# ethan-li-coding/AD-Census

Hardware: AMD Instinct MI355X
Metric: stereo pairs/s at 1920x1080 D=128 (ADCensusStereo::Match, images and disparity map resident in HBM) (higher is better)
Workload: dtype f32; 1 GPU; noise 1920x1080 D=128 (BASELINE.json configs[3]); batch=160 distinct pairs (seeds 12345+i), 668 per GPU (cycled), queue=static round-robin partition, in_flight_per_gpu=1, parallelism=replicas x1 (independent pairs), full=False

## Files before the change

adcensus_amd/__init__.py:

```python
import ctypes as C
import os

import numpy as np

_HERE = os.path.dirname(os.path.abspath(__file__))
LIB_PATH = os.environ.get("ADC_HIP_LIB") or os.path.join(_HERE, "lib", "libadcensus_hip.so")

STAGES = ["cost", "arms", "aggregate", "scanline", "wta", "refine"]
(BUF_GRAY_LEFT, BUF_GRAY_RIGHT, BUF_CENSUS_LEFT, BUF_CENSUS_RIGHT, BUF_ARMS, BUF_SUPCOUNT_H, BUF_SUPCOUNT_V,
 BUF_VOLUME_A, BUF_DISP_LEFT, BUF_DISP_RIGHT, BUF_OUTLIER_LABEL) = range(11)
(RUN_GRAY_CENSUS, RUN_COST, RUN_ARMS, RUN_AGGREGATE, RUN_SCANLINE, RUN_WTA, RUN_LRCHECK, RUN_REGION_VOTING,
 RUN_INTERPOLATION, RUN_DISCONTINUITY, RUN_MEDIAN) = range(11)
MAX_DISP_RANGE = 2047
PAPER_CENSUS5X5, PAPER_SO_SUM, PAPER_RIGHT_ARMS = 1, 2, 4
LR_CONSISTENT, LR_MISMATCH, LR_OCCLUSION = 0, 1, 2
FILL_WTA, FILL_VOTING, FILL_INTERPOLATION, FILL_NONE = 0, 1, 2, 3
PROV_LR_MASK, PROV_FILL_SHIFT = 3, 2
PROV_SPECKLE = 0x10
PIX_BGR8, PIX_RGB8, PIX_GRAY8, PIX_BGRA8 = 0, 1, 2, 3
PIX_GRAY16 = 0x10
PIX_BAYER_RGGB8, PIX_BAYER_GRBG8, PIX_BAYER_GBRG8, PIX_BAYER_BGGR8 = 0x20, 0x21, 0x22, 0x23
PIX_BAYER_RGGB16, PIX_BAYER_GRBG16, PIX_BAYER_GBRG16, PIX_BAYER_BGGR16 = 0x30, 0x31, 0x32, 0x33
PIX_YUYV, PIX_UYVY, PIX_NV12 = 0x40, 0x41, 0x42
PIX_BYTES = {PIX_BGR8: 3, PIX_RGB8: 3, PIX_GRAY8: 1, PIX_BGRA8: 4, PIX_GRAY16: 2, PIX_YUYV: 2, PIX_UYVY: 2, PIX_NV12: 1,
# ... 325 lines not shown
    L.adc_get_aggregate_info.restype = C.c_int
    L.adc_get_aggregate_kernel.argtypes = [vp]
    L.adc_get_aggregate_kernel.restype = C.c_char_p
    L.adc_host_register.argtypes = [vp, C.c_size_t]
    L.adc_host_register.restype = C.c_int
    L.adc_host_unregister.argtypes = [vp]
    L.adc_host_unregister.restype = C.c_int
    L.adc_set_paper_modes.argtypes = [vp, C.c_uint32]
    L.adc_set_paper_modes.restype = C.c_int
    L.adc_get_stream.argtypes = [vp]
    L.adc_get_stream.restype = vp
    L.adc_device_synchronize.restype = C.c_int
    L.adc_device_malloc.argtypes = [C.c_size_t]
    L.adc_device_malloc.restype = vp
    L.adc_device_free.argtypes = [vp]
    L.adc_device_free.restype = None
    L.adc_memcpy_h2d.argtypes = [vp, vp, C.c_size_t]
    L.adc_memcpy_h2d.restype = C.c_int
    L.adc_memcpy_d2h.argtypes = [vp, vp, C.c_size_t]
    L.adc_memcpy_d2h.restype = C.c_int
    L.adc_device_copy_ms.argtypes = [vp, vp, C.c_size_t, C.c_int]
    L.adc_device_copy_ms.restype = C.c_double
    if hasattr(L, "adc_device_copy_kernel_ms"):
        L.adc_device_copy_kernel_ms.argtypes = [vp, vp, C.c_size_t, C.c_int]
        L.adc_device_copy_kernel_ms.restype = C.c_double
    L.adc_debug_read.argtypes = [vp, C.c_int, vp]
    L.adc_debug_read.restype = C.c_int
    L.adc_debug_write.argtypes = [vp, C.c_int, vp]
    L.adc_debug_write.restype = C.c_int
    L.adc_debug_set_images.argtypes = [vp, u8p, u8p]
    L.adc_debug_set_images.restype = C.c_int
    L.adc_debug_run.argtypes = [vp, C.c_int, C.c_int]
    L.adc_debug_run.restype = C.c_int
    L.adc_farm_create.argtypes = [i32, i32, C.POINTER(ADCensusOption), C.c_int, C.c_int]
    L.adc_farm_create.restype = vp
    L.adc_farm_destroy.argtypes = [vp]
    L.adc_farm_destroy.restype = None
    L.adc_farm_submit.argtypes = [vp, u8p, u8p, vp, C.POINTER(C.c_uint64)]
    L.adc_farm_submit.restype = C.c_int
    L.adc_farm_wait.argtypes = [vp, C.c_uint64]
    L.adc_farm_wait.restype = C.c_int
    L.adc_farm_drain.argtypes = [vp]
    L.adc_farm_drain.restype = C.c_int64
    L.adc_debug_counter.argtypes = [vp, C.c_int]
    L.adc_debug_counter.restype = C.c_int64
    L.adc_debug_voting_stats.argtypes = [vp, C.POINTER(C.c_int64), C.POINTER(C.c_int64)]
    L.adc_debug_voting_stats.restype = C.c_int
    _lib = L
    return L


def device_count():
    return lib().adc_device_count()


def last_error():
    return lib().adc_last_error().decode()


def host_register(arr):
    if lib().adc_host_register(arr.ctypes.data, arr.nbytes) != 0:
        raise RuntimeError("adc_host_register failed: " + last_error())


def host_unregister(arr):
    lib().adc_host_unregister(arr.ctypes.data)
# ... 523 lines not shown
            raise RuntimeError("adc_set_paper_modes failed: " + last_error())

    def aggregate_kernel(self):
        return lib().adc_get_aggregate_kernel(self._h).decode()

    def _buf_spec(self, which):
        h, w, d = self.height, self.width, self.disp_range
        return {
            BUF_GRAY_LEFT: (np.uint8, (h, w)), BUF_GRAY_RIGHT: (np.uint8, (h, w)),
            BUF_CENSUS_LEFT: (np.uint64, (h, w)), BUF_CENSUS_RIGHT: (np.uint64, (h, w)),
            BUF_ARMS: (np.uint8, (h, w, 4)),
            BUF_SUPCOUNT_H: (np.uint16, (h, w)), BUF_SUPCOUNT_V: (np.uint16, (h, w)),
            BUF_VOLUME_A: (np.float32, (h, w, d)),
            BUF_DISP_LEFT: (np.float32, (h, w)), BUF_DISP_RIGHT: (np.float32, (h, w)),
            BUF_OUTLIER_LABEL: (np.uint8, (h, w)),
        }[which]

    def debug_read(self, which):
        dt, shp = self._buf_spec(which)
        out = np.empty(shp, dtype=dt)
        rc = lib().adc_debug_read(self._h, which, out.ctypes.data)
        if rc != 0:
            raise RuntimeError("adc_debug_read(%d) failed: %s" % (which, last_error()))
        return out

    def debug_write(self, which, arr):
        dt, shp = self._buf_spec(which)
        a = np.ascontiguousarray(arr, dtype=dt)
        assert a.shape == tuple(shp), (a.shape, shp)
        rc = lib().adc_debug_write(self._h, which, a.ctypes.data)
        if rc != 0:
            raise RuntimeError("adc_debug_write(%d) failed: %s" % (which, last_error()))

    def debug_set_images(self, img_left, img_right):
        l, r = _img(img_left), _img(img_right)
        if lib().adc_debug_set_images(self._h, l.ctypes.data, r.ctypes.data) != 0:
            raise RuntimeError("adc_debug_set_images failed: " + last_error())

    def debug_run(self, stage, arg=0):
        rc = lib().adc_debug_run(self._h, stage, arg)
        if rc != 0:
            raise RuntimeError("adc_debug_run(%d) failed: %s" % (stage, last_error()))

    def debug_set_budget(self, kernels):
        rc = lib().adc_debug_run(self._h, RUN_REGION_VOTING, -int(kernels))
        if rc != 0:
            raise RuntimeError("adc_debug_run failed: " + last_error())

    def debug_counter(self, which):
        return int(lib().adc_debug_counter(self._h, which))

    def voting_stats(self):
        r, e = C.c_int64(0), C.c_int64(0)
        lib().adc_debug_voting_stats(self._h, C.byref(r), C.byref(e))
        return int(r.value), int(e.value)
```

adcensus_amd/csrc/capi.hip:

```cpp
#include "adc_internal.h"
#include "adc_device_fn.h"
#include "itp_plan.h"

#include <math.h>
#include <stdio.h>
#include <stdlib.h>
#include <string.h>
#include <string>
#include <vector>
#include <new>
#include <mutex>
#include <atomic>

static thread_local std::string g_last_error;

#ifdef ADC_FAULT_INJECTION
static std::atomic<long> g_fi_calls{0};
static std::atomic<long> g_fi_fail_at{[] { const char* e = getenv("ADC_TEST_FAIL_AT"); return e ? atol(e) : 0L; }()};
extern "C" int adc_test_fault_now(void) { const long n = ++g_fi_calls; return n == g_fi_fail_at.load(); }
extern "C" void adc_test_fail_at(long n) { g_fi_calls = 0; g_fi_fail_at = n; }
extern "C" long adc_test_hip_calls(void) { return g_fi_calls.load(); }
static std::atomic<long> g_fi_live{0};
extern "C" long adc_test_live_buffers(void) { return g_fi_live.load(); }
#define ADC_LIVE(d) (g_fi_live += (d))
// ... 1847 lines not shown
    case ADC_BUF_DISP_LEFT: return {h->disp_l, P * 4, false};
    case ADC_BUF_DISP_RIGHT: return {h->disp_r, P * 4, false};
    case ADC_BUF_OUTLIER_LABEL: return {h->label, P, false};
    default: return {nullptr, 0, false};
    }
}

int adc_debug_read(adc_handle* h, int which, void* dst)
{
    if (!h || !dst) return 1;
    hipSetDevice(h->device);
    const BufDesc b = buf_desc(h, which);
    if (!b.ptr) return 1;
    if (b.volume) {
        if (adc_launch_unpad_volume(h, h->vol_a, h->vol_b) != hipSuccess) return 2;
        if (hipMemcpyAsync(dst, h->vol_b, b.bytes, hipMemcpyDeviceToHost, h->stream) != hipSuccess) return 2;
    } else if (hipMemcpyAsync(dst, b.ptr, b.bytes, hipMemcpyDeviceToHost, h->stream) != hipSuccess) return 2;
    return hipStreamSynchronize(h->stream) == hipSuccess ? 0 : 2;
}

int adc_debug_write(adc_handle* h, int which, const void* src)
{
    if (!h || !src) return 1;
    hipSetDevice(h->device);
    const BufDesc b = buf_desc(h, which);
    if (!b.ptr) return 1;
    if (b.volume) {
        if (hipMemcpyAsync(h->vol_b, src, b.bytes, hipMemcpyHostToDevice, h->stream) != hipSuccess) return 2;
        if (adc_launch_pad_volume(h, h->vol_b, h->vol_a) != hipSuccess) return 2;
    } else if (hipMemcpyAsync(b.ptr, src, b.bytes, hipMemcpyHostToDevice, h->stream) != hipSuccess) return 2;
    return hipStreamSynchronize(h->stream) == hipSuccess ? 0 : 2;
}

int adc_debug_set_images(adc_handle* h, const uint8_t* left, const uint8_t* right)
{
    if (!h || !left || !right) return 1;
    hipSetDevice(h->device);
    const size_t P = (size_t)h->p.W * h->p.H;
    images_own(h, true);
    if (hipMemcpy(h->img_l, left, P * 3, hipMemcpyHostToDevice) != hipSuccess) return 2;
    if (hipMemcpy(h->img_r, right, P * 3, hipMemcpyHostToDevice) != hipSuccess) return 2;
    return 0;
}

int adc_debug_run(adc_handle* h, int stage, int arg)
{
    if (!h) return 1;
    hipSetDevice(h->device);
    hipError_t e = hipSuccess;
    bool fuse_cost = false; AggArms arms = AGG_ARMS_UNKNOWN;
    switch (stage) {
    case ADC_RUN_GRAY_CENSUS: e = adc_launch_gray_census(h); break;
    case ADC_RUN_COST: e = adc_launch_cost(h, h->vol_a); break;
    case ADC_RUN_ARMS: e = adc_launch_arms(h); break;
    case ADC_RUN_AGGREGATE:
        e = hipMemsetAsync(h->armmax + ADC_NZ_BASE, 0, 2 * ADC_NZ_SHARDS * ADC_NZ_STRIDE * sizeof(int), h->heavy);
        if (e == hipSuccess) e = adc_launch_records(h);
        if (e == hipSuccess && arg >= 200) {
            int am[2] = {0, 0};
            e = hipMemcpy(am, h->armmax, 2 * sizeof(int), hipMemcpyDeviceToHost);
            if (e == hipSuccess) learn_take_arms(&h->learned, am);
            if (e == hipSuccess) arms = AGG_ARMS_EXACT;
            if (e == hipSuccess && h->pin_nz) e = hipMemcpyAsync(h->pin_nz, h->armmax + ADC_NZ_BASE, 2 * ADC_NZ_SHARDS * ADC_NZ_STRIDE * sizeof(int32_t), hipMemcpyDeviceToHost, h->heavy);
            if (e == hipSuccess && h->pin_nz) e = hipStreamSynchronize(h->heavy);
            if (e == hipSuccess && h->pin_nz) {
                long long nz[2];
// ... 108 lines not shown
```

adcensus_amd/csrc/k_refine.hip:

```cpp
#include "adc_internal.h"
#include <mutex>
#include "adc_device_fn.h"
#include "itp_plan.h"

#include <vector>
#include <stdio.h>
#include <stdlib.h>

__device__ __forceinline__ bool lr_invalid(const float* __restrict__ dl, const float* __restrict__ dr, int W, int x, int y,
                                           float thres, int& col_right, float& disp_r)
{
    const float d = dl[(size_t)y * W + x];
    col_right = -1;
    disp_r = 0.f;
    if (d == ADC_INVALID_FLOAT) return true;
    const long cr = lroundf((float)x - d);
    if (cr < 0 || cr >= W) return true;
    col_right = (int)cr;
    disp_r = dr[(size_t)y * W + cr];
    return fabsf(d - disp_r) > thres;
}

__global__ __launch_bounds__(256) void k_lr_phase1(const float* __restrict__ dl, const float* __restrict__ dr,
                                                   uint8_t* __restrict__ inv, int W, int H, float thres)
// ... 157 lines not shown
        if (mismatch) {
            int key = (hit != ADC_INVALID_FLOAT && dist < 9999) ? dist * 16 + s : 0x7fffffff;
            float val = hit;
#pragma unroll
            for (int msk = 8; msk >= 1; msk >>= 1) {
                const int ok = __shfl_xor(key, msk, 64);
                const float ov = __shfl_xor(val, msk, 64);
                if (ok < key) { key = ok; val = ov; }
            }
            unsigned long long hb = __ballot(hit != ADC_INVALID_FLOAT);
            any = ((hb >> (lane & 48)) & 0xffffull) != 0;
            best = key != 0x7fffffff ? val : 0.0f;
        } else {
            float val = hit;
#pragma unroll
            for (int msk = 8; msk >= 1; msk >>= 1) {
                const float ov = __shfl_xor(val, msk, 64);
                val = ov < val ? ov : val;
            }
            any = val != ADC_INVALID_FLOAT;
            best = val;
        }
        if (live && s == 0) dout[e] = any ? best : 0.0f;
    }
}

__global__ void k_pack_bgr(const uint8_t* __restrict__ img, uint32_t* __restrict__ out, int P);
__device__ __forceinline__ int packed_l1(uint32_t a, uint32_t b)
{
    return (int)__builtin_amdgcn_sad_u8(a, b, 0u);
}

#define ITP_CELL ADC_ITP_CELL
static size_t itp_cell_stride(int W, int H) { return adc_itp_cell_stride(W, H); }
static size_t itp_code_offset(int W, int H) { return adc_itp_code_offset(W, H); }
static size_t itp_code_stride(int W, int H, int ms) { return adc_itp_code_stride(W, H, ms); }
__device__ __forceinline__ bool itp_valid(const float* __restrict__ disp, const uint8_t* __restrict__ label, size_t p, int pass2)
{
    return disp[p] != ADC_INVALID_FLOAT || (pass2 && label[p] == ADC_LABEL_MISMATCH);
}
__global__ __launch_bounds__(256) void k_itp_cells(const float* __restrict__ disp, const uint8_t* __restrict__ label, uint8_t* __restrict__ cell, int W, int H, int cw, int ch, size_t map_stride)
{
    const int c = blockIdx.x * 256 + threadIdx.x;
    if (c >= cw * ch) return;
    const int cy = c / cw, cx = c - cy * cw;
    bool any = false;
#pragma unroll
    for (int r = 0; r < ITP_CELL; r++)
#pragma unroll
        for (int q = 0; q < ITP_CELL; q++) {
            const int y = cy * ITP_CELL + r, x = cx * ITP_CELL + q;
            if (y < H && x < W) any = any || itp_valid(disp, label, (size_t)y * W + x, (int)blockIdx.y);
        }
    cell[blockIdx.y * map_stride + c] = any ? 1 : 0;
}
__global__ __launch_bounds__(256) void k_itp_rowdist(const uint8_t* __restrict__ cell, uint8_t* __restrict__ rowd, int cw, int ch, size_t map_stride)
{
    const int c = blockIdx.x * 256 + threadIdx.x;
    if (c >= cw * ch) return;
    rowd[blockIdx.y * map_stride + c] = (uint8_t)adc_itp_rowdist(cell + blockIdx.y * map_stride, cw, c % cw, c / cw);
}
__global__ __launch_bounds__(256) void k_itp_coldist(const uint8_t* __restrict__ rowd, uint8_t* __restrict__ cdist, int cw, int ch, size_t map_stride)
{
    const int c = blockIdx.x * 256 + threadIdx.x;
    if (c >= cw * ch) return;
    cdist[blockIdx.y * map_stride + c] = (uint8_t)adc_itp_coldist(rowd + blockIdx.y * map_stride, cw, ch, c % cw, c / cw);
}

__global__ __launch_bounds__(256) void k_itp_code(const float* __restrict__ disp, const uint8_t* __restrict__ label, const uint8_t* __restrict__ cdist,
                                                  uint8_t* __restrict__ code, int W, int H, int cw, int pitch, int gx, size_t cell_stride, size_t code_stride)
{
    cdist += blockIdx.y * cell_stride;
    code += blockIdx.y * code_stride;
    const int i = blockIdx.x * 256 + threadIdx.x;
    const int q4 = (W + 3) >> 2;
    if (i >= q4 * H + H) return;
    const int y = i / (q4 + 1), k = i - y * (q4 + 1);
    const int c0 = (gx & ~3) + 4 * k;
    uint32_t v = 0u;
#pragma unroll
    for (int b = 0; b < 4; b++) {
        const int x = c0 + b - gx;
        uint32_t c = ADC_ITP_OUTSIDE;
        if (x >= 0 && x < W) c = itp_valid(disp, label, (size_t)y * W + x, (int)blockIdx.y) ? (uint32_t)ADC_ITP_VALID : (uint32_t)adc_itp_skip(cdist[(y / ITP_CELL) * cw + (x / ITP_CELL)]);
        v |= c << (8 * b);
    }
    *reinterpret_cast<uint32_t*>(code + (size_t)y * pitch + c0) = v;
}

template <int N>
__device__ __forceinline__ void itp_trip(const int32_t* __restrict__ lt, const uint8_t* __restrict__ code, uint32_t pb, int s, int max_search,
                                         bool& walking, int& m, int& ho)
{
    const bool w0 = walking && m < max_search;
    uint32_t c[N];
    int o[N];
#pragma unroll
    for (int j = 0; j < N; j++) { c[j] = ADC_ITP_OUTSIDE; o[j] = 0; }
    if (w0) {
        const int32_t* row = lt + (m * 16 + s);
#pragma unroll
        for (int j = 0; j < N; j++) { o[j] = row[j * 16]; c[j] = code[pb + (uint32_t)o[j]]; }
    }
    bool act = w0;
    const int left = max_search - m;
#pragma unroll
    for (int j = 0; j < N; j++) {
        const bool end = c[j] >= ADC_ITP_OUTSIDE || j >= left;
        ho = (act && end && c[j] == ADC_ITP_VALID && j < left) ? o[j] : ho;
        act = act && !end;
    }
    walking = act;
    m += act ? N + (int)c[N - 1] : 0;
}
#define ITP_NO_HIT 0x7fffffff
#ifndef ITP_NS1
#define ITP_NS1 2
#endif
#ifndef ITP_NS2
#define ITP_NS2 4
// ... 117 lines not shown
                    if (ok < key) { key = ok; val = ov; }
                }
                any = key != 0x7fffffff;
                best = any ? val : 0.0f;
            } else {
                float val = hit;
#pragma unroll
                for (int msk = 32; msk >= 4; msk >>= 1) {
                    const float ov = __shfl_xor(val, msk, 64);
                    val = ov < val ? ov : val;
                }
                any = val != ADC_INVALID_FLOAT;
                best = val;
            }
            if (live[k] && s == 0) dmap[p[k]] = any ? best : 0.0f;
        }
    }
}

__global__ __launch_bounds__(256) void k_interp_scatter(const int32_t* __restrict__ list, const int32_t* __restrict__ counters,
                                                        const float* __restrict__ fill, float* __restrict__ disp)
{
    const int n = counters[0];
    for (int e = blockIdx.x * 256 + threadIdx.x; e < n; e += gridDim.x * 256) disp[list[e]] = fill[e];
}

hipError_t adc_launch_interpolation(adc_handle* h, bool force_f64)
{
    const AdcParams& p = h->p;
    const int P = p.W * p.H;
    const int dmaxa = p.dmax < 0 ? -p.dmax : p.dmax, dmina = p.dmin < 0 ? -p.dmin : p.dmin;
    const int max_search = dmaxa > dmina ? dmaxa : dmina;
    if (h->ray_tab && !force_f64 && max_search == h->ray_tab_rows && max_search == h->itp_ms && adc_itp_table_walk_ok(p.W, p.H, h->itp_ms)) {
        hipError_t e;
        if ((e = hipMemsetAsync(h->interp_counters, 0, 8 * sizeof(int32_t), h->stream)) != hipSuccess) return e;
        hipLaunchKernelGGL(k_interp_list2, dim3((P + 256 * ITP_LIST_PPT - 1) / (256 * ITP_LIST_PPT)), dim3(256), 0, h->stream, h->label, h->disp_l,
                           h->interp_list, h->interp_list + P, h->interp_counters, P);
        if (!h->bgrx_valid) hipLaunchKernelGGL(k_pack_bgr, dim3((P + 255) / 256), dim3(256), 0, h->stream, h->img_l, h->bgrx_l, P);
        const int cw = (p.W + ITP_CELL - 1) / ITP_CELL, ch = (p.H + ITP_CELL - 1) / ITP_CELL, nc = cw * ch;
        const size_t cs = itp_cell_stride(p.W, p.H), ks = itp_code_stride(p.W, p.H, h->itp_ms);
        uint8_t* code = h->itp_cells + itp_code_offset(p.W, p.H);
        hipLaunchKernelGGL(k_itp_cells, dim3((nc + 255) / 256, 2), dim3(256), 0, h->stream, h->disp_l, h->label, h->itp_cells, p.W, p.H, cw, ch, cs);
        hipLaunchKernelGGL(k_itp_rowdist, dim3((nc + 255) / 256, 2), dim3(256), 0, h->stream, h->itp_cells, h->itp_cells + nc, cw, ch, cs);
        hipLaunchKernelGGL(k_itp_coldist, dim3((nc + 255) / 256, 2), dim3(256), 0, h->stream, h->itp_cells + nc, h->itp_cells + 2 * nc, cw, ch, cs);
        hipLaunchKernelGGL(k_itp_code, dim3((((p.W + 3) / 4 + 1) * p.H + 255) / 256, 2), dim3(256), 0, h->stream, h->disp_l, h->label, h->itp_cells + 2 * (size_t)nc,
                           code, p.W, p.H, cw, h->itp_pitch, h->itp_ms, cs, ks);
        const size_t lin_bytes = (size_t)(max_search + ADC_ITP_LPAD) * 16 * sizeof(int32_t);
        const bool tab_lds = lin_bytes <= 40 * 1024;
        for (int k = 0; k < 2; k++) {
            const int which = k == 0 ? ADC_LABEL_MISMATCH : ADC_LABEL_OCCLUSION;
#define INTERP_TAB(L_)                                                                                                 \
    hipLaunchKernelGGL((k_interpolate_tab<L_>), dim3(2048), dim3(256), L_ ? lin_bytes : 0, h->stream, h->interp_list + (size_t)k * P, h->interp_counters + k, \
                       h->disp_l, h->bgrx_l, h->ray_lin, p.W, which, max_search, code + k * ks, h->itp_pitch, h->itp_ms, 1.0f / (float)h->itp_pitch)
            if (tab_lds) INTERP_TAB(true);
            else INTERP_TAB(false);
#undef INTERP_TAB
        }
        return hipGetLastError();
    }
    for (int k = 0; k < 2; k++) {
        const int which = k == 0 ? ADC_LABEL_MISMATCH : ADC_LABEL_OCCLUSION;
        hipError_t e;
        if ((e = hipMemsetAsync(h->interp_counters, 0, 8 * sizeof(int32_t), h->stream)) != hipSuccess) return e;
        hipLaunchKernelGGL(k_interp_list, dim3((P + 256 * ITP_LIST_PPT - 1) / (256 * ITP_LIST_PPT)), dim3(256), 0, h->stream, h->label, h->disp_l,
                           h->interp_list, h->interp_counters, which, P);
        hipLaunchKernelGGL(k_interpolate_rays, dim3(2048), dim3(256), 0, h->stream, h->interp_list, h->interp_counters, h->disp_l,
                           h->disp_tmp, h->img_l, h->ray_sincos, p.W, p.H, which, max_search);
        hipLaunchKernelGGL(k_interp_scatter, dim3(1024), dim3(256), 0, h->stream, h->interp_list, h->interp_counters, h->disp_tmp, h->disp_l);
    }
    return hipGetLastError();
}

__global__ __launch_bounds__(256) void k_edge_detect(const float* __restrict__ dp, uint8_t* __restrict__ edge, int W, int H,
                                                     float threshold)
{
    const int x = blockIdx.x * 64 + (threadIdx.x & 63);
    const int y = blockIdx.y * 4 + (threadIdx.x >> 6);
    if (x >= W || y >= H) return;
    uint8_t e = 0;
// ... 526 lines not shown
```

adcensus_amd/csrc/k_scanline.hip:

```cpp
#include "adc_internal.h"
#include "adc_device_fn.h"

template <int CTRL>
__device__ __forceinline__ float dpp_mov(float old, float src)
{
    return __int_as_float(__builtin_amdgcn_update_dpp(__float_as_int(old), __float_as_int(src), CTRL, 0xf, 0xf, false));
}

template <bool DPP>
__device__ __forceinline__ float wave_min_f32(float v)
{
    if constexpr (DPP) {
        asm("s_nop 1\n\tv_min_f32_dpp %0, %0, %0 row_ror:1 row_mask:0xf bank_mask:0xf\n\t"
            "s_nop 1\n\tv_min_f32_dpp %0, %0, %0 row_ror:2 row_mask:0xf bank_mask:0xf\n\t"
            "s_nop 1\n\tv_min_f32_dpp %0, %0, %0 row_ror:4 row_mask:0xf bank_mask:0xf\n\t"
            "s_nop 1\n\tv_min_f32_dpp %0, %0, %0 row_ror:8 row_mask:0xf bank_mask:0xf\n\t"
            "s_nop 1\n\tv_min_f32_dpp %0, %0, %0 row_bcast:15 row_mask:0xa bank_mask:0xf\n\t"
            "s_nop 1\n\tv_min_f32_dpp %0, %0, %0 row_bcast:31 row_mask:0xc bank_mask:0xf\n\t"
            "s_nop 1"
            : "+v"(v));
        return __int_as_float(__builtin_amdgcn_readlane(__float_as_int(v), 63));
    } else {
#pragma unroll
        for (int m = 32; m >= 1; m >>= 1) {
// ... 224 lines not shown
    const int plen_v = e1 - e0;
    g.d0 = lane * VPL;
    const uint32_t* c1p = c1w + (size_t)g.path * ngr;
    const int cl_last = g.d0 + VPL - 1 + dmin;

    float agr[AGG ? 2 * SO_AGG_LA + 1 : 1][VPL];
    const uint32_t* recp = AGG ? aggrec + (size_t)g.path * W : nullptr;
#define SO_AGG_PUSH(C)                                                                                         \
    do {                                                                                                       \
        _Pragma("unroll") for (int t_ = 2 * SO_AGG_LA; t_ > 0; t_--)                                           \
            _Pragma("unroll") for (int k_ = 0; k_ < VPL; k_++) agr[t_][k_] = agr[t_ - 1][k_];                  \
        _Pragma("unroll") for (int k_ = 0; k_ < VPL; k_++) agr[0][k_] = (C)[k_];                               \
    } while (0)
#define SO_AGG_EVAL(EIDX, C)                                                                                   \
    do {                                                                                                       \
        const uint32_t rec_ = recp[(EIDX)];                                                                    \
         \
         \
         \
         \
        if (!adc_rec_changes_pixel(rec_, true)) {                                                              \
            _Pragma("unroll") for (int k_ = 0; k_ < VPL; k_++) (C)[k_] = agr[SO_AGG_LA][k_];                   \
        } else {                                                                                               \
            const int top_ = SO_AGG_LA + (int)(rec_ & 255u), bot_ = SO_AGG_LA - (int)((rec_ >> 8) & 255u);     \
            const float cnt_ = (float)(rec_ >> 16);                                                            \
            _Pragma("unroll") for (int k_ = 0; k_ < VPL; k_++) {                                               \
                float acc_ = 0.0f;                                                                             \
                _Pragma("unroll") for (int t_ = 2 * SO_AGG_LA; t_ >= 0; t_--) acc_ += (t_ <= top_ && t_ >= bot_) ? agr[t_][k_] : 0.0f; \
                (C)[k_] = acc_ / cnt_;                               \
            }                                                                                                  \
        }                                                                                                      \
    } while (0)
    float Lp[VPL];
    float minLp;
    {
        const size_t pix = so_pixel<VERT>(g, e0);
        float c[VPL];
        if constexpr (AGG) {
#pragma unroll
            for (int t_ = 0; t_ <= 2 * SO_AGG_LA; t_++) {
                const int er_ = adc_imax(0, adc_imin(g.plen - 1, e0 + SO_AGG_LA - t_));
                vload<VPL>(src + so_pixel<VERT>(g, er_) * Dp + g.d0, agr[t_]);
            }
            SO_AGG_EVAL(e0, c);
        } else
        vload<VPL>(src + pix * Dp + g.d0, c);
        if (!SEG || seg == 0) vstore<VPL>(dst + pix * Dp + g.d0, c);
        float lmin = ADC_LARGE_FLOAT;
#pragma unroll
        for (int k = 0; k < VPL; k++) {
            Lp[k] = (g.d0 + k) < D ? c[k] : ADC_LARGE_FLOAT;
            lmin = Lp[k] < lmin ? Lp[k] : lmin;
        }
        minLp = wave_min_f32<DPP>(lmin);
    }
    float upN = lane_up<DPP>(Lp[VPL - 1], ADC_LARGE_FLOAT, lane);
    float dnN = lane_down<DPP>(Lp[0], ADC_LARGE_FLOAT, lane);
    int wtaB = 0;
    float wtaC1 = 0.f, wtaC2 = 0.f, wtaM = 0.f;
#define SO_WTA(I)                                                                                          \
    if constexpr (WTA) {                                                                                   \
        int bi_ = 0x7fffffff;                                                                              \
        _Pragma("unroll") for (int k = 0; k < VPL; k++)                                                    \
        {                                                                                                  \
            const unsigned long long m_ = __ballot(Lp[k] == minLp);                                        \
            const int c_ = m_ ? (int)__builtin_ctzll(m_) * VPL + k : 0x7fffffff;                           \
            bi_ = c_ < bi_ ? c_ : bi_;                                                                     \
        }                                                                                                  \
         \
        const int best_ = minLp < ADC_LARGE_FLOAT ? bi_ + dmin : 0;                                        \
         \
        const int idx_ = (best_ - dmin) & (64 * VPL - 1);                                                  \
        const int kw_ = idx_ % VPL, lw_ = idx_ / VPL;                                                      \
        float s1_ = upN, s2_ = VPL == 1 ? dnN : Lp[VPL == 1 ? 0 : 1];                                      \
        _Pragma("unroll") for (int k = 1; k < VPL; k++)                                                    \
        {                                                                                                  \
            s1_ = kw_ == k ? Lp[k - 1] : s1_;                                                              \
            s2_ = kw_ == k ? (k == VPL - 1 ? dnN : Lp[k == VPL - 1 ? k : k + 1]) : s2_;                    \
        }                                                                                                  \
        const int c1_ = __builtin_amdgcn_readlane(__float_as_int(s1_), lw_);                               \
        const int c2_ = __builtin_amdgcn_readlane(__float_as_int(s2_), lw_);                               \
        const int slot_ = (I)&63;                                                                          \
        const bool mine_ = lane == slot_;                        \
        wtaB = mine_ ? best_ : wtaB;                                                                       \
        wtaC1 = mine_ ? __int_as_float(c1_) : wtaC1;                                                       \
        wtaC2 = mine_ ? __int_as_float(c2_) : wtaC2;                                                       \
        wtaM = mine_ ? minLp : wtaM;                                                                       \
        if (slot_ == 63 || (I) == g.plen - 1) {                                                            \
            const int e_ = ((I) & ~63) + lane;                       \
            if (e_ <= (I)) {                                                                               \
                float o_;                                                                                  \
                if (wtaB == dmin || wtaB == dmin + D - 1) o_ = ADC_INVALID_FLOAT;                          \
                else if (wtaB - 1 - dmin < 0 || wtaB + 1 - dmin >= D) o_ = (float)wtaB;                    \
                else o_ = adc_subpixel(wtaB, wtaC1, wtaC2, wtaM);                                          \
                disp[so_pixel<VERT>(g, e_)] = o_;                                                          \
            }                                                                                              \
        }                                                                                                  \
    }
    SO_WTA(0);
    if (plen_v <= 1) return;

    int mcur = dir > 0 ? e0 + 1 : g.plen - 2 - e0;
    const int dpad = (D + VPL - 1) / VPL * VPL;
#define SO_STEP(I, E)                                                                                      \
    do {                                                                                                   \
        const int x_ = VERT ? g.path : mcur;    \
        int off_[VPL];                                                                                     \
        if (SO_INTERIOR && adc_so_interior(x_, W, dmin, dpad))  \
            adc_so_class_offsets_interior<VPL>((E).rb, (E).c1, tso, off_);                                 \
        else                                                                                               \
            adc_so_class_offsets<VPL>((E).rb, (E).c1, x_ - cl_last, W, tso, W >= 3 && x_ - dmin >= 1, off_);   \
        const float up_ = upN;                                           \
        const float dn_ = dnN;                                          \
        float out_[VPL];                                                                                   \
        _Pragma("unroll") for (int k = 0; k < VPL; k++)                                                    \
        {                                                                                                  \
            const float2 pp_ = *reinterpret_cast<const float2*>(reinterpret_cast<const char*>(so_tab) + off_[k]); \
            const float P1_ = pp_.x, P2_ = pp_.y;                                                          \
            const float lm1_ = k == 0 ? up_ : Lp[k == 0 ? 0 : k - 1];                                      \
            const float lp1_ = k == VPL - 1 ? dn_ : Lp[k == VPL - 1 ? k : k + 1];                          \
            const float l1_ = Lp[k];                                                                       \
            const float l2_ = lm1_ + P1_;                                                                  \
            const float l3_ = lp1_ + P1_;                                                                  \
            const float l4_ = minLp + P2_;                                                                 \
               \
            const float mm_ = __builtin_fminf(__builtin_fminf(__builtin_fminf(l1_, l2_), l3_), l4_);       \
            float cs_ = (E).c[k] + mm_;                                                                    \
            cs_ = cs_ * 0.5f;                          \
            out_[k] = cs_;                                                                                 \
        }                                                                                                  \
        SO_STORE(I, out_);                                                                                 \
        float omin_ = ADC_LARGE_FLOAT;                                                                     \
        _Pragma("unroll") for (int k = 0; k < VPL; k++)                                                    \
        {                                                                                                  \
            Lp[k] = (g.d0 + k) < D ? out_[k] : ADC_LARGE_FLOAT;                                            \
            omin_ = __builtin_fminf(Lp[k], omin_);                                                         \
        }                                                                                                  \
        minLp = wave_min_f32<DPP>(omin_);                                                                  \
        upN = lane_up<DPP>(Lp[VPL - 1], ADC_LARGE_FLOAT, lane);                                            \
        dnN = lane_down<DPP>(Lp[0], ADC_LARGE_FLOAT, lane);                                                \
        SO_WTA(I);                                                                                         \
        mcur += dir;                                                                                       \
    } while (0)
#define SO_STORE(I, OUT)              \
    do {                              \
        vstore<VPL>(dpn, OUT);        \
        dpn += dstep;                 \
    } while (0)
#define SO_STEP_F(I, E)                                                                                    \
    do {                                                                                                   \
        int off_[VPL];                                                                                     \
        adc_so_class_offsets_interior<VPL>((E).rb, (E).c1, tso, off_);                                     \
        float out_[VPL];                                                                                   \
        _Pragma("unroll") for (int k = 0; k < VPL; k++)                                                    \
        {                                                                                                  \
            const float2 pp_ = *reinterpret_cast<const float2*>(reinterpret_cast<const char*>(so_tab) + off_[k]); \
            const float lm1_ = k == 0 ? upN : Lp[k == 0 ? 0 : k - 1];                                      \
            const float lp1_ = k == VPL - 1 ? dnN : Lp[k == VPL - 1 ? k : k + 1];                          \
            const float l2_ = lm1_ + pp_.x;                                                                \
            const float l3_ = lp1_ + pp_.x;                                                                \
            const float l4_ = minLp + pp_.y;                                                               \
            float t_, mm_;                                                                                 \
            asm("v_min3_f32 %0, %1, %2, %3" : "=v"(t_) : "v"(Lp[k]), "v"(l2_), "v"(l3_));                  \
            asm("v_min_f32 %0, %1, %2" : "=v"(mm_) : "v"(t_), "v"(l4_));                                   \
            out_[k] = ((E).c[k] + mm_) * 0.5f;                                                             \
        }                                                                                                  \
        SO_STORE(I, out_);                                                                                 \
        float omin_ = out_[0];                                                                             \
        _Pragma("unroll") for (int k = 0; k < VPL; k++) Lp[k] = out_[k];                                   \
        if constexpr (VPL == 2) asm("v_min_f32 %0, %1, %2" : "=v"(omin_) : "v"(out_[0]), "v"(out_[1]));    \
        minLp = wave_min_f32<DPP>(omin_);                                                                  \
        if constexpr (DPP) {                                                                               \
            upN = dpp_mov<0x138>(upN, Lp[VPL - 1]);                                                        \
            dnN = dpp_mov<0x130>(dnN, Lp[0]);                                                              \
        } else {                                                                                           \
            upN = lane_up<DPP>(Lp[VPL - 1], ADC_LARGE_FLOAT, lane);                                        \
            dnN = lane_down<DPP>(Lp[0], ADC_LARGE_FLOAT, lane);                                            \
        }                                                                                                  \
        SO_WTA(I);                                                                                         \
    } while (0)

    if constexpr (VPL <= 2) {
        typedef typename VecT<VPL>::type vec_t;
        constexpr int PF = 16, NG = PF / 4;
        if constexpr (PIN) asm volatile("" ::: SO_CLOBBERS);
        vec_t pfc[PIN ? 1 : PF];
        uint32_t pfr[PIN ? 1 : PF];
        uint32_t pfw[PIN ? 1 : NG];
        const long long pstep = (long long)(VERT ? W : 1) * dir;
        const long long fstep = pstep * Dp;
        const size_t px1 = so_pixel<VERT>(g, e0 + 1);
        const float* spn = src + (AGG ? so_pixel<VERT>(g, adc_imin(e0 + 1 + SO_AGG_LA, g.plen - 1)) : px1) * Dp + g.d0;
        const uint32_t* cwn = c1p + (e0 >> 2);
        float* dpn = dst + px1 * Dp + g.d0;
        long long dstep = fstep;
        if constexpr (SEG) {
            if (seg > 0) {
                dpn = seam + ((size_t)g.path * (nseg - 1) + (seg - 1)) * Dp + g.d0;
                dstep = 0;
            }
        }
        const int last = e1 - 1;
        int ii = e0 + 1, gi = e0 >> 2;
        int mpf = mcur;
#define SO_ISSUE_D(U)                                                                                          \
    do {                                                                                                       \
        const int ro_ = so_rmap_offset_m<VPL, VERT>(g, mpf, cl_last);                                          \
        if constexpr (PIN) {                                                                                   \
            if constexpr (VPL == 1) {                                                                          \
                asm volatile("global_load_dword v[%1], %0, off" ADC_VOL_NT_STR ::"v"(spn), "n"(SO_RC(U)) : "memory");         \
                asm volatile("global_load_ubyte v[%2], %0, %1" ::"v"(ro_), "s"(rmap), "n"(SO_RR(U)) : "memory"); \
            } else {                                                                                           \
// ... 456 lines not shown
```

include/adcensus_c_api.h:

```cpp
#ifndef ADCENSUS_C_API_H_
#define ADCENSUS_C_API_H_

#include <stdint.h>
#include <stddef.h>

#ifdef __cplusplus
extern "C" {
#endif

typedef struct adc_option {
    int32_t min_disparity;
    int32_t max_disparity;
    int32_t lambda_ad;
    int32_t lambda_census;
    int32_t cross_L1;
    int32_t cross_L2;
    int32_t cross_t1;
    int32_t cross_t2;
    float   so_p1;
    float   so_p2;
    int32_t so_tso;
    int32_t irv_ts;
    float   irv_th;
    float   lrcheck_thres;
// ... 235 lines not shown

#define ADC_PAPER_CENSUS5X5 1u
#define ADC_PAPER_SO_SUM 2u
#define ADC_PAPER_RIGHT_ARMS 4u
int adc_set_paper_modes(adc_handle* h, uint32_t modes);

void adc_set_verbose(adc_handle* h, int on);

void* adc_get_stream(adc_handle* h);
int   adc_device_synchronize(void);
void* adc_device_malloc(size_t bytes);
void  adc_device_free(void* p);
int   adc_memcpy_h2d(void* dst, const void* src, size_t bytes);
int   adc_memcpy_d2h(void* dst, const void* src, size_t bytes);
double adc_device_copy_ms(void* dst, const void* src, size_t bytes, int reps);
double adc_device_copy_kernel_ms(void* dst, const void* src, size_t bytes, int reps);

enum {
    ADC_BUF_GRAY_LEFT = 0,
    ADC_BUF_GRAY_RIGHT,
    ADC_BUF_CENSUS_LEFT,
    ADC_BUF_CENSUS_RIGHT,
    ADC_BUF_ARMS,
    ADC_BUF_SUPCOUNT_H,
    ADC_BUF_SUPCOUNT_V,
    ADC_BUF_VOLUME_A,
    ADC_BUF_DISP_LEFT,
    ADC_BUF_DISP_RIGHT,
    ADC_BUF_OUTLIER_LABEL,
    ADC_BUF_COUNT
};
int adc_debug_read(adc_handle* h, int which, void* dst);
int adc_debug_write(adc_handle* h, int which, const void* src);
int adc_debug_set_images(adc_handle* h, const uint8_t* bgr_left, const uint8_t* bgr_right);

enum {
    ADC_RUN_GRAY_CENSUS = 0,
    ADC_RUN_COST,
    ADC_RUN_ARMS,
    ADC_RUN_AGGREGATE,
    ADC_RUN_SCANLINE,
    ADC_RUN_WTA,
    ADC_RUN_LRCHECK,
    ADC_RUN_REGION_VOTING,
    ADC_RUN_INTERPOLATION,
    ADC_RUN_DISCONTINUITY,
    ADC_RUN_MEDIAN,
    ADC_RUN_COUNT
};
int adc_debug_run(adc_handle* h, int stage, int arg);
int64_t adc_debug_counter(adc_handle* h, int which);
int adc_debug_voting_stats(adc_handle* h, int64_t* rounds, int64_t* evaluations);

#ifdef __cplusplus
}
#endif
#endif
```

Before: 333.1 pairs/s.

## Fuse interpolation code-map setup into one tiled kernel and streamline scanline WTA

Replaces the memset plus four interpolation setup kernels (cells, row distance, column distance, code) with one tiled kernel. That kernel computes cell validity with ballots, row and column distances in LDS, and writes the code map for both passes while also zeroing the counters. The scanline fused winner-take-all is also reworked: it uses a single ballot on the per-lane minimum and selects neighbours with one pass, writes slot values with v_writelane, and tracks the flush point with a counter. Debug API entries to read the code maps are added. The intent is to cut launch overhead and global traffic in refinement and to trim per-step WTA work, at the cost of halo redundancy and subtle tie-break semantics.

```diff
diff --git a/adcensus_amd/__init__.py b/adcensus_amd/__init__.py
--- a/adcensus_amd/__init__.py
+++ b/adcensus_amd/__init__.py
@@ -381,6 +381,11 @@
     L.adc_debug_set_images.restype = C.c_int
     L.adc_debug_run.argtypes = [vp, C.c_int, C.c_int]
     L.adc_debug_run.restype = C.c_int
+    if hasattr(L, "adc_debug_read_itp_code"):
+        L.adc_debug_itp_code_geometry.argtypes = [vp, C.POINTER(C.c_int), C.POINTER(C.c_int), C.POINTER(C.c_int)]
+        L.adc_debug_itp_code_geometry.restype = C.c_int
+        L.adc_debug_read_itp_code.argtypes = [vp, C.c_int, vp]
+        L.adc_debug_read_itp_code.restype = C.c_int
     L.adc_farm_create.argtypes = [i32, i32, C.POINTER(ADCensusOption), C.c_int, C.c_int]
     L.adc_farm_create.restype = vp
     L.adc_farm_destroy.argtypes = [vp]
@@ -970,6 +975,16 @@
         if rc != 0:
             raise RuntimeError("adc_debug_write(%d) failed: %s" % (which, last_error()))
 
+    def debug_read_itp_code(self, which_pass):
+        pitch, rows, gx = C.c_int(0), C.c_int(0), C.c_int(0)
+        if lib().adc_debug_itp_code_geometry(self._h, C.byref(pitch), C.byref(rows), C.byref(gx)) != 0:
+            raise RuntimeError("adc_debug_itp_code_geometry failed: " + last_error())
+        out = np.empty((rows.value, pitch.value), dtype=np.uint8)
+        rc = lib().adc_debug_read_itp_code(self._h, int(which_pass), out.ctypes.data)
+        if rc != 0:
+            raise RuntimeError("adc_debug_read_itp_code(%d) failed: %s" % (which_pass, last_error()))
+        return out, gx.value
+
     def debug_set_images(self, img_left, img_right):
         l, r = _img(img_left), _img(img_right)
         if lib().adc_debug_set_images(self._h, l.ctypes.data, r.ctypes.data) != 0:
diff --git a/adcensus_amd/csrc/capi.hip b/adcensus_amd/csrc/capi.hip
--- a/adcensus_amd/csrc/capi.hip
+++ b/adcensus_amd/csrc/capi.hip
@@ -1903,6 +1903,26 @@
     return hipStreamSynchronize(h->stream) == hipSuccess ? 0 : 2;
 }
 
+int adc_debug_itp_code_geometry(adc_handle* h, int* pitch, int* rows, int* gx)
+{
+    if (!h || !pitch || !rows || !gx) return 1;
+    if (h->itp_pitch == 0) { g_last_error = "adc_debug_itp_code_geometry: this handle has no code maps (itp_plan.h)"; return 1; }
+    *pitch = h->itp_pitch;
+    *rows = adc_itp_code_rows(h->p.H, h->itp_ms);
+    *gx = h->itp_ms;
+    return 0;
+}
+
+int adc_debug_read_itp_code(adc_handle* h, int pass, void* dst)
+{
+    int pitch, rows, gx;
+    if (!dst || pass < 0 || pass > 1 || adc_debug_itp_code_geometry(h, &pitch, &rows, &gx) != 0) return 1;
+    hipSetDevice(h->device);
+    const uint8_t* code = h->itp_cells + adc_itp_code_offset(h->p.W, h->p.H) + (size_t)pass * adc_itp_code_stride(h->p.W, h->p.H, h->itp_ms);
+    if (hipMemcpyAsync(dst, code, (size_t)pitch * rows, hipMemcpyDeviceToHost, h->stream) != hipSuccess) return 2;
+    return hipStreamSynchronize(h->stream) == hipSuccess ? 0 : 2;
+}
+
 int adc_debug_set_images(adc_handle* h, const uint8_t* left, const uint8_t* right)
 {
     if (!h || !left || !right) return 1;
diff --git a/adcensus_amd/csrc/k_refine.hip b/adcensus_amd/csrc/k_refine.hip
--- a/adcensus_amd/csrc/k_refine.hip
+++ b/adcensus_amd/csrc/k_refine.hip
@@ -213,60 +213,87 @@
 }
 
 #define ITP_CELL ADC_ITP_CELL
-static size_t itp_cell_stride(int W, int H) { return adc_itp_cell_stride(W, H); }
 static size_t itp_code_offset(int W, int H) { return adc_itp_code_offset(W, H); }
 static size_t itp_code_stride(int W, int H, int ms) { return adc_itp_code_stride(W, H, ms); }
-__device__ __forceinline__ bool itp_valid(const float* __restrict__ disp, const uint8_t* __restrict__ label, size_t p, int pass2)
-{
-    return disp[p] != ADC_INVALID_FLOAT || (pass2 && label[p] == ADC_LABEL_MISMATCH);
-}
-__global__ __launch_bounds__(256) void k_itp_cells(const float* __restrict__ disp, const uint8_t* __restrict__ label, uint8_t* __restrict__ cell, int W, int H, int cw, int ch, size_t map_stride)
-{
-    const int c = blockIdx.x * 256 + threadIdx.x;
-    if (c >= cw * ch) return;
-    const int cy = c / cw, cx = c - cy * cw;
-    bool any = false;
-#pragma unroll
-    for (int r = 0; r < ITP_CELL; r++)
-#pragma unroll
-        for (int q = 0; q < ITP_CELL; q++) {
-            const int y = cy * ITP_CELL + r, x = cx * ITP_CELL + q;
-            if (y < H && x < W) any = any || itp_valid(disp, label, (size_t)y * W + x, (int)blockIdx.y);
-        }
-    cell[blockIdx.y * map_stride + c] = any ? 1 : 0;
-}
-__global__ __launch_bounds__(256) void k_itp_rowdist(const uint8_t* __restrict__ cell, uint8_t* __restrict__ rowd, int cw, int ch, size_t map_stride)
-{
-    const int c = blockIdx.x * 256 + threadIdx.x;
-    if (c >= cw * ch) return;
-    rowd[blockIdx.y * map_stride + c] = (uint8_t)adc_itp_rowdist(cell + blockIdx.y * map_stride, cw, c % cw, c / cw);
-}
-__global__ __launch_bounds__(256) void k_itp_coldist(const uint8_t* __restrict__ rowd, uint8_t* __restrict__ cdist, int cw, int ch, size_t map_stride)
-{
-    const int c = blockIdx.x * 256 + threadIdx.x;
-    if (c >= cw * ch) return;
-    cdist[blockIdx.y * map_stride + c] = (uint8_t)adc_itp_coldist(rowd + blockIdx.y * map_stride, cw, ch, c % cw, c / cw);
-}
-
-__global__ __launch_bounds__(256) void k_itp_code(const float* __restrict__ disp, const uint8_t* __restrict__ label, const uint8_t* __restrict__ cdist,
-                                                  uint8_t* __restrict__ code, int W, int H, int cw, int pitch, int gx, size_t cell_stride, size_t code_stride)
-{
-    cdist += blockIdx.y * cell_stride;
-    code += blockIdx.y * code_stride;
-    const int i = blockIdx.x * 256 + threadIdx.x;
+#define ITP_T_DW 14
+#define ITP_T_CX (ITP_T_DW * 4 / ITP_CELL + 2)
+#define ITP_T_CR 64
+#define ITP_T_HR (ITP_T_CR + 2 * ADC_ITP_CAP)
+#define ITP_T_WAVES 16
+static_assert(ITP_CELL == 2 && ADC_ITP_CAP == 16 && ITP_T_CX + 2 * ADC_ITP_CAP <= 64 && ITP_T_CX <= 32 && ITP_T_CR * 32 == 2048 && ITP_T_HR % ITP_T_WAVES == 0, "k_itp_setup: one lane per cell column, shifts below");
+__global__ __launch_bounds__(64 * ITP_T_WAVES) void k_itp_setup(const float* __restrict__ disp, const uint8_t* __restrict__ label, uint8_t* __restrict__ code,
+                                                                int W, int H, int pitch, int gx, size_t code_stride, int32_t* __restrict__ counters)
+{
+    __shared__ uint8_t rowd[2][ITP_T_HR][32];
+    __shared__ uint8_t pixv[ITP_T_CR][32];
+    __shared__ uint8_t skip[2][ITP_T_CR][32];
+    const int lane = threadIdx.x & 63, wave = threadIdx.x >> 6;
+    if (blockIdx.x == 0 && blockIdx.y == 0 && threadIdx.x < 8) counters[threadIdx.x] = 0;
+    const int cx0 = (int)blockIdx.x * (ITP_T_DW * 2) - 2 - ADC_ITP_CAP;
+    const int cy0 = (int)blockIdx.y * ITP_T_CR - ADC_ITP_CAP;
+    const int x0 = (cx0 + lane) * ITP_CELL;
+    constexpr int NR = ITP_T_HR / ITP_T_WAVES;
+    float dv[NR][ITP_CELL * ITP_CELL];
+    uint8_t lv[NR][ITP_CELL * ITP_CELL];
+#pragma unroll
+    for (int j = 0; j < NR; j++)
+#pragma unroll
+        for (int t = 0; t < ITP_CELL * ITP_CELL; t++) {
+            const int y = (cy0 + wave + j * ITP_T_WAVES) * ITP_CELL + t / ITP_CELL, x = x0 + t % ITP_CELL;
+            const size_t p = ((unsigned)x < (unsigned)W && (unsigned)y < (unsigned)H) ? (size_t)y * W + x : 0;
+            dv[j][t] = disp[p];
+            lv[j][t] = label[p];
+        }
+#pragma unroll
+    for (int j = 0; j < NR; j++) {
+        const int lr = wave + j * ITP_T_WAVES;
+        uint32_t bits = 0u;
+#pragma unroll
+        for (int t = 0; t < ITP_CELL * ITP_CELL; t++) {
+            const int y = (cy0 + lr) * ITP_CELL + t / ITP_CELL, x = x0 + t % ITP_CELL;
+            const bool in = (unsigned)x < (unsigned)W && (unsigned)y < (unsigned)H;
+            const bool inv = dv[j][t] == ADC_INVALID_FLOAT, mis = lv[j][t] == ADC_LABEL_MISMATCH;
+            bits |= (in && !inv ? 1u : 0u) << t | (in && (!inv || mis) ? 1u : 0u) << (4 + t);
+        }
+        const unsigned long long m[2] = {__ballot((bits & 15u) != 0u), __ballot(bits != 0u)};
+        if (lane >= ADC_ITP_CAP && lane < ADC_ITP_CAP + 32) {
+#pragma unroll
+            for (int k = 0; k < 2; k++) {
+                const uint32_t lo = (uint32_t)(m[k] >> (lane - ADC_ITP_CAP)) & 0x1ffffu;
+                const uint32_t hi = (uint32_t)(m[k] >> lane) & 0x1ffffu;
+                const int dl = lo ? __clz((int)lo) - 15 : ADC_ITP_CAP + 1, dr = hi ? __ffs((int)hi) - 1 : ADC_ITP_CAP + 1;
+                rowd[k][lr][lane - ADC_ITP_CAP] = (uint8_t)adc_imin(dl, dr);
+            }
+            if (lr >= ADC_ITP_CAP && lr < ADC_ITP_CAP + ITP_T_CR) pixv[lr - ADC_ITP_CAP][lane - ADC_ITP_CAP] = (uint8_t)bits;
+        }
+    }
+    __syncthreads();
+    for (int i = threadIdx.x; i < 2 * ITP_T_CR * 32; i += 64 * ITP_T_WAVES) {
+        const int col = i & 31, row = (i >> 5) & (ITP_T_CR - 1), k = i >> 11;
+        int best = ADC_ITP_CAP + 1;
+        for (int dy = 0; dy <= ADC_ITP_CAP && dy < best; dy++)
+            best = adc_imin(best, adc_imax(adc_imin((int)rowd[k][row + ADC_ITP_CAP - dy][col], (int)rowd[k][row + ADC_ITP_CAP + dy][col]), dy));
+        skip[k][row][col] = (uint8_t)adc_itp_skip(best);
+    }
+    __syncthreads();
     const int q4 = (W + 3) >> 2;
-    if (i >= q4 * H + H) return;
-    const int y = i / (q4 + 1), k = i - y * (q4 + 1);
-    const int c0 = (gx & ~3) + 4 * k;
-    uint32_t v = 0u;
-#pragma unroll
-    for (int b = 0; b < 4; b++) {
-        const int x = c0 + b - gx;
-        uint32_t c = ADC_ITP_OUTSIDE;
-        if (x >= 0 && x < W) c = itp_valid(disp, label, (size_t)y * W + x, (int)blockIdx.y) ? (uint32_t)ADC_ITP_VALID : (uint32_t)adc_itp_skip(cdist[(y / ITP_CELL) * cw + (x / ITP_CELL)]);
-        v |= c << (8 * b);
-    }
-    *reinterpret_cast<uint32_t*>(code + (size_t)y * pitch + c0) = v;
+    for (int i = threadIdx.x; i < 2 * ITP_T_CR * ITP_CELL * ITP_T_DW; i += 64 * ITP_T_WAVES) {
+        const int kl = i % ITP_T_DW, r = (i / ITP_T_DW) & (ITP_T_CR * ITP_CELL - 1), pass = i / (ITP_T_DW * ITP_T_CR * ITP_CELL);
+        const int k = (int)blockIdx.x * ITP_T_DW + kl, y = (int)blockIdx.y * (ITP_T_CR * ITP_CELL) + r;
+        if (k > q4 || y >= H) continue;
+        uint32_t v = 0u;
+#pragma unroll
+        for (int b = 0; b < 4; b++) {
+            const int x = 4 * k + b - (gx & 3);
+            uint32_t c = ADC_ITP_OUTSIDE;
+            if ((unsigned)x < (unsigned)W) {
+                const int lc = (x >> 1) - (cx0 + ADC_ITP_CAP), lrow = r >> 1;
+                c = ((pixv[lrow][lc] >> (pass * 4 + (r & 1) * 2 + (x & 1))) & 1) ? (uint32_t)ADC_ITP_VALID : (uint32_t)skip[pass][lrow][lc];
+            }
+            v |= c << (8 * b);
+        }
+        *reinterpret_cast<uint32_t*>(code + pass * code_stride + (size_t)y * pitch + (gx & ~3) + 4 * k) = v;
+    }
 }
 
 template <int N>
@@ -450,19 +477,13 @@
     const int dmaxa = p.dmax < 0 ? -p.dmax : p.dmax, dmina = p.dmin < 0 ? -p.dmin : p.dmin;
     const int max_search = dmaxa > dmina ? dmaxa : dmina;
     if (h->ray_tab && !force_f64 && max_search == h->ray_tab_rows && max_search == h->itp_ms && adc_itp_table_walk_ok(p.W, p.H, h->itp_ms)) {
-        hipError_t e;
-        if ((e = hipMemsetAsync(h->interp_counters, 0, 8 * sizeof(int32_t), h->stream)) != hipSuccess) return e;
+        const size_t ks = itp_code_stride(p.W, p.H, h->itp_ms);
+        uint8_t* code = h->itp_cells + itp_code_offset(p.W, p.H);
+        hipLaunchKernelGGL(k_itp_setup, dim3((((p.W + 3) >> 2) + 1 + ITP_T_DW - 1) / ITP_T_DW, (p.H + ITP_T_CR * ITP_CELL - 1) / (ITP_T_CR * ITP_CELL)), dim3(64 * ITP_T_WAVES), 0,
+                           h->stream, h->disp_l, h->label, code, p.W, p.H, h->itp_pitch, h->itp_ms, ks, h->interp_counters);
         hipLaunchKernelGGL(k_interp_list2, dim3((P + 256 * ITP_LIST_PPT - 1) / (256 * ITP_LIST_PPT)), dim3(256), 0, h->stream, h->label, h->disp_l,
                            h->interp_list, h->interp_list + P, h->interp_counters, P);
         if (!h->bgrx_valid) hipLaunchKernelGGL(k_pack_bgr, dim3((P + 255) / 256), dim3(256), 0, h->stream, h->img_l, h->bgrx_l, P);
-        const int cw = (p.W + ITP_CELL - 1) / ITP_CELL, ch = (p.H + ITP_CELL - 1) / ITP_CELL, nc = cw * ch;
-        const size_t cs = itp_cell_stride(p.W, p.H), ks = itp_code_stride(p.W, p.H, h->itp_ms);
-        uint8_t* code = h->itp_cells + itp_code_offset(p.W, p.H);
-        hipLaunchKernelGGL(k_itp_cells, dim3((nc + 255) / 256, 2), dim3(256), 0, h->stream, h->disp_l, h->label, h->itp_cells, p.W, p.H, cw, ch, cs);
-        hipLaunchKernelGGL(k_itp_rowdist, dim3((nc + 255) / 256, 2), dim3(256), 0, h->stream, h->itp_cells, h->itp_cells + nc, cw, ch, cs);
-        hipLaunchKernelGGL(k_itp_coldist, dim3((nc + 255) / 256, 2), dim3(256), 0, h->stream, h->itp_cells + nc, h->itp_cells + 2 * nc, cw, ch, cs);
-        hipLaunchKernelGGL(k_itp_code, dim3((((p.W + 3) / 4 + 1) * p.H + 255) / 256, 2), dim3(256), 0, h->stream, h->disp_l, h->label, h->itp_cells + 2 * (size_t)nc,
-                           code, p.W, p.H, cw, h->itp_pitch, h->itp_ms, cs, ks);
         const size_t lin_bytes = (size_t)(max_search + ADC_ITP_LPAD) * 16 * sizeof(int32_t);
         const bool tab_lds = lin_bytes <= 40 * 1024;
         for (int k = 0; k < 2; k++) {
diff --git a/adcensus_amd/csrc/k_scanline.hip b/adcensus_amd/csrc/k_scanline.hip
--- a/adcensus_amd/csrc/k_scanline.hip
+++ b/adcensus_amd/csrc/k_scanline.hip
@@ -280,7 +280,7 @@
         }                                                                                                      \
     } while (0)
     float Lp[VPL];
-    float minLp;
+    float minLp, lmin0;
     {
         const size_t pix = so_pixel<VERT>(g, e0);
         float c[VPL];
@@ -301,40 +301,47 @@
             lmin = Lp[k] < lmin ? Lp[k] : lmin;
         }
         minLp = wave_min_f32<DPP>(lmin);
+        lmin0 = lmin;
     }
     float upN = lane_up<DPP>(Lp[VPL - 1], ADC_LARGE_FLOAT, lane);
     float dnN = lane_down<DPP>(Lp[0], ADC_LARGE_FLOAT, lane);
     int wtaB = 0;
     float wtaC1 = 0.f, wtaC2 = 0.f, wtaM = 0.f;
-#define SO_WTA(I)                                                                                          \
+    int wtaNext = adc_imin(63, g.plen - 1);
+#define SO_WTA(I, LM)                                                                                      \
     if constexpr (WTA) {                                                                                   \
-        int bi_ = 0x7fffffff;                                                                              \
-        _Pragma("unroll") for (int k = 0; k < VPL; k++)                                                    \
+        const unsigned long long m_ = __ballot((LM) == minLp);                                             \
+        const int lw_ = (int)__builtin_ctzll(m_);    \
+        int kw_ = VPL - 1;                                                                                 \
+        float s1_ = VPL == 1 ? upN : Lp[VPL == 1 ? 0 : VPL - 2], s2_ = dnN;                                \
+        bool e0_ = true;                                                                                   \
+        _Pragma("unroll") for (int k = VPL - 2; k >= 0; k--)                                               \
         {                                                                                                  \
-            const unsigned long long m_ = __ballot(Lp[k] == minLp);                                        \
-            const int c_ = m_ ? (int)__builtin_ctzll(m_) * VPL + k : 0x7fffffff;                           \
-            bi_ = c_ < bi_ ? c_ : bi_;                                                                     \
+            const bool e_ = Lp[k] == minLp;                                                                \
+            if (VPL > 2) kw_ = e_ ? k : kw_;                                                               \
+            s1_ = e_ ? (k == 0 ? upN : Lp[k == 0 ? 0 : k - 1]) : s1_;                                      \
+            s2_ = e_ ? Lp[k + 1 < VPL ? k + 1 : k] : s2_;                                                  \
+            e0_ = e_;                                                                                      \
         }                                                                                                  \
-         \
-        const int best_ = minLp < ADC_LARGE_FLOAT ? bi_ + dmin : 0;                                        \
-         \
-        const int idx_ = (best_ - dmin) & (64 * VPL - 1);                                                  \
-        const int kw_ = idx_ % VPL, lw_ = idx_ / VPL;                                                      \
-        float s1_ = upN, s2_ = VPL == 1 ? dnN : Lp[VPL == 1 ? 0 : 1];                                      \
-        _Pragma("unroll") for (int k = 1; k < VPL; k++)                                                    \
-        {                                                                                                  \
-            s1_ = kw_ == k ? Lp[k - 1] : s1_;                                                              \
-            s2_ = kw_ == k ? (k == VPL - 1 ? dnN : Lp[k == VPL - 1 ? k : k + 1]) : s2_;                    \
-        }                                                                                                  \
+                 \
+        const int kk_ = VPL == 1 ? 0 : (VPL == 2 ? (int)((~__ballot(e0_) >> lw_) & 1ull) : __builtin_amdgcn_readlane(kw_, lw_)); \
         const int c1_ = __builtin_amdgcn_readlane(__float_as_int(s1_), lw_);                               \
         const int c2_ = __builtin_amdgcn_readlane(__float_as_int(s2_), lw_);                               \
+         \
+         \
+         \
+                                         \
+        const int best_ = __float_as_int(minLp) < __float_as_int(ADC_LARGE_FLOAT) ? lw_ * VPL + kk_ + dmin : 0; \
         const int slot_ = (I)&63;                                                                          \
-        const bool mine_ = lane == slot_;                        \
-        wtaB = mine_ ? best_ : wtaB;                                                                       \
-        wtaC1 = mine_ ? __int_as_float(c1_) : wtaC1;                                                       \
-        wtaC2 = mine_ ? __int_as_float(c2_) : wtaC2;                                                       \
-        wtaM = mine_ ? minLp : wtaM;                                                                       \
-        if (slot_ == 63 || (I) == g.plen - 1) {                                                            \
+         \
+                                                                     \
+        asm("s_mov_b32 m0, %4\n\tv_writelane_b32 %0, %5, m0\n\tv_writelane_b32 %1, %6, m0\n\t"             \
+            "v_writelane_b32 %2, %7, m0\n\tv_writelane_b32 %3, %8, m0"                                     \
+            : "+v"(wtaB), "+v"(wtaC1), "+v"(wtaC2), "+v"(wtaM)                                             \
+            : "s"(slot_), "s"(best_), "s"(c1_), "s"(c2_), "s"(minLp)                                       \
+            : "m0");                                                                                       \
+        if ((I) == wtaNext) {                                         \
+            wtaNext = adc_imin(wtaNext + 64, g.plen - 1);                                                  \
             const int e_ = ((I) & ~63) + lane;                       \
             if (e_ <= (I)) {                                                                               \
                 float o_;                                                                                  \
@@ -345,7 +352,7 @@
             }                                                                                              \
         }                                                                                                  \
     }
-    SO_WTA(0);
+    SO_WTA(0, lmin0);
     if (plen_v <= 1) return;
 
     int mcur = dir > 0 ? e0 + 1 : g.plen - 2 - e0;
@@ -387,7 +394,7 @@
         minLp = wave_min_f32<DPP>(omin_);                                                                  \
         upN = lane_up<DPP>(Lp[VPL - 1], ADC_LARGE_FLOAT, lane);                                            \
         dnN = lane_down<DPP>(Lp[0], ADC_LARGE_FLOAT, lane);                                                \
-        SO_WTA(I);                                                                                         \
+        SO_WTA(I, omin_);                                                                                  \
         mcur += dir;                                                                                       \
     } while (0)
 #define SO_STORE(I, OUT)              \
@@ -425,7 +432,7 @@
             upN = lane_up<DPP>(Lp[VPL - 1], ADC_LARGE_FLOAT, lane);                                        \
             dnN = lane_down<DPP>(Lp[0], ADC_LARGE_FLOAT, lane);                                            \
         }                                                                                                  \
-        SO_WTA(I);                                                                                         \
+        SO_WTA(I, omin_);                                                                                  \
     } while (0)
 
     if constexpr (VPL <= 2) {
diff --git a/include/adcensus_c_api.h b/include/adcensus_c_api.h
--- a/include/adcensus_c_api.h
+++ b/include/adcensus_c_api.h
@@ -291,6 +291,8 @@
 };
 int adc_debug_read(adc_handle* h, int which, void* dst);
 int adc_debug_write(adc_handle* h, int which, const void* src);
+int adc_debug_itp_code_geometry(adc_handle* h, int* pitch, int* rows, int* gx);
+int adc_debug_read_itp_code(adc_handle* h, int pass, void* dst);
 int adc_debug_set_images(adc_handle* h, const uint8_t* bgr_left, const uint8_t* bgr_right);
 
 enum {
```

After: 340.4 pairs/s, median of 6. 1.02x the previous value.
